# tmuird/VAEUNET

Measured on AMD Instinct MI355X. Metric: images/sec (whole node) at 3x512x512 bs=8/GPU; Dice parity vs CPU ref, higher is better.
Workload: dtype bf16; 1 GPU; UNet(3,2) train step (fwd+CombinedLoss+bwd+clip+AdamW), random-init weights; image=3x512x512, batch_per_gpu=8, global_batch=8, parallelism=dp1, execution=hipgraph-replay, wgrad_side_stream=False

## Files before the change

include/vaeunet.h:

```cpp
#ifndef VAEUNET_H
#define VAEUNET_H
#include <stdint.h>
#ifdef __cplusplus
extern "C" {
#endif

typedef struct VuGather {
  const void* src[3];
  int64_t stride[3];
  int32_t cend[3];
  int32_t nsrc;
  int32_t C;
  int32_t N, H, W;
  int32_t Hs, Ws;
  int32_t R, S;
  int32_t sy, sx, dy, dx, oy, ox;
} VuGather;

typedef struct VuGemmFwd {
  VuGather a;
  const void* b;
  int64_t ldb;
  int32_t ncol;
  int32_t out_mode;
// ... 121 lines not shown
int64_t vu_permute4_chunk(void);
int64_t vu_permute4_tile(void);
int vu_permute4_batch(const VuPermJob* jobs, int njobs, int64_t nchunks,
                      void* stream);
int vu_permute4_batch2(const VuPermJob* jobs, int njobs, int ntap,
                       int64_t tap_blocks, int64_t rest_blocks, void* stream);

int vu_bn_finalize(const float* psum, const float* pm2, int tiles,
                   int64_t tile_rows, int64_t rows, int C,
                   const float* gamma, const float* beta,
                   float* running_mean, float* running_var, float momentum,
                   float eps, float* scale, float* shift, float* save_mean,
                   float* save_invstd, int64_t* num_batches_tracked,
                   float* workspace, void* stream);
int vu_bn_eval_coeffs(const float* gamma, const float* beta,
                      const float* running_mean, const float* running_var,
                      float eps, int C, float* scale, float* shift,
                      float* save_mean, float* save_invstd, void* stream);
int vu_bn_fwd_fused_supported(int tiles, int C, int64_t ys, int64_t rs, int64_t os);
int vu_bn_fwd_fused(const float* psum, const float* pm2, int tiles, int64_t tile_rows, int64_t P, int C,
                    const float* gamma, const float* beta, float* running_mean, float* running_var,
                    int64_t* num_batches_tracked, float momentum, float eps, float* coef, const void* y,
                    int64_t ys, const void* res, int64_t rs, const float* rscale, const float* rshift,
                    void* out, int64_t os, int relu, int dtype, void* stream);
int vu_bn_apply(const void* x, int64_t x_stride, void* y, int64_t y_stride,
                int64_t P, int C, const float* scale, const float* shift,
                int relu, int dtype, void* stream);
int vu_bn_bwd_fused_supported(int64_t P, int C, int64_t dys, int64_t xs, int64_t dxs);
int vu_bn_bwd_fused(const void* dy, int64_t dys, const void* x, int64_t xs, int64_t P, int C,
                    const float* scale, const float* shift, const float* mean, const float* invstd,
                    const float* gamma, int relu, int train, float* dgamma, float* dbeta,
                    int accumulate, void* dx, int64_t dxs, float* workspace, int dtype, void* stream);
int vu_bn_bwd_reduce(const void* dy, int64_t dy_stride, const void* x,
                     int64_t x_stride, int64_t P, int C, const float* scale,
                     const float* shift, const float* mean,
                     const float* invstd, const float* gamma, int relu,
                     int train, float* dgamma, float* dbeta, int accumulate,
                     float* coef, float* workspace, int dtype, void* stream);
int64_t vu_bn_bwd_finish_workspace_bytes(int nblk, int C);
int vu_bn_bwd_finish(const float* part, int nblk, int64_t P, int C,
                     const float* gamma, const float* invstd, int train,
                     float* dgamma, float* dbeta, int accumulate, float* coef,
                     float* workspace, void* stream);
int vu_bn_bwd_apply(const void* dy, int64_t dy_stride, const void* x,
                    int64_t x_stride, int64_t P, int C, const float* scale,
                    const float* shift, const float* mean, const float* coef,
                    int relu, void* dx, int64_t dx_stride, int dtype,
                    void* stream);
int vu_bn_bwd_apply2_ok(int C, int64_t dys, int64_t x1s, int64_t x2s, int64_t dx1s, int64_t dx2s);
int vu_bn_bwd_apply2(const void* dy, int64_t dys, const void* x1, int64_t x1s, const void* x2, int64_t x2s,
                     int64_t P, int C, const float* mean1, const float* coef1, const float* mean2,
                     const float* coef2, void* dx1, int64_t dx1s, void* dx2, int64_t dx2s, int dtype,
                     void* stream);

int vu_chan_sum(const void* x, int64_t stride, int N, int H, int W, int y0,
                int x0, int Hr, int Wr, int C, float* out, int accumulate,
                float* workspace, int dtype, void* stream);
int64_t vu_reduce_workspace_bytes(int64_t P, int C);
int64_t vu_bn_finalize_workspace_bytes(int tiles, int C);
int vu_zero(void* y, int64_t ys, int64_t P, int C, int dtype, void* stream);
int vu_gpu_delay(int rounds, void* stream);
int vu_zero_insert2(const void* dy, int64_t dys, int N, int h, int w, int C,
                    void* up, int64_t ups, int H, int W, int dtype, void* stream);
int vu_copy(const void* x, int64_t xs, int xdtype, void* y, int64_t ys,
            int ydtype, int64_t P, int C, int accumulate, void* stream);
int vu_input_pack(const float* x, int64_t sn, int64_t sc, int64_t sh,
                  int64_t sw, int N, int C, int H, int W, int Cp, void* y,
                  int dtype, void* stream);

int vu_maxpool2_fwd(const void* x, int64_t xs, int N, int H, int W, int C,
                    void* y, int64_t ys, int dtype, void* stream);
int vu_maxpool2_bwd(const void* x, int64_t xs, const void* dy, int64_t dys,
                    int N, int H, int W, int C, void* dx, int64_t dxs,
                    const void* add, int64_t adds, int dtype, void* stream);
int vu_bn_apply_maxpool2(const void* y, int64_t ys, void* a, int64_t as, void* pool, int64_t ps,
                         int N, int H, int W, int C, const float* scale, const float* shift,
                         int relu, int dtype, void* stream);
int vu_bn_bwd_pool_supported(int H, int W, int C, int64_t ys, int64_t dps, int64_t adds, int64_t dxs);
int vu_bn_bwd_pool(const void* y, int64_t ys, const void* dp, int64_t dps, const void* add, int64_t adds,
                   int N, int H, int W, int C, const float* scale, const float* shift, const float* mean,
                   const float* invstd, const float* gamma, int relu, int train, float* dgamma,
                   float* dbeta, int accumulate, float* coef, float* workspace, void* dx, int64_t dxs,
                   int dtype, void* stream);
int vu_upsample_fwd(const void* x, int64_t xs, int N, int Hi, int Wi, int C,
                    void* y, int64_t ys, int Ho, int Wo, int Hp, int Wp,
                    int py, int px, int dtype, void* stream);
int vu_upsample_bwd(const void* dy, int64_t dys, int N, int Hi, int Wi, int C,
                    void* dx, int64_t dxs, int Ho, int Wo, int Hp, int Wp,
                    int py, int px, int accumulate, int dtype, void* stream);

int64_t vu_attn_tile_rows(void);
int vu_attn_psi_fwd(const void* ug, const void* ux, int64_t P, int F,
                    const float* sg, const float* tg, const float* sx,
                    const float* tx, const float* wpsi, const float* bpsi,
                    float* q, float* psum, float* pm2, int64_t tile_rows,
                    int dtype, void* stream);
int vu_attn_gate_fwd(const float* q, const float* st, const void* x,
                     int64_t xs, int64_t P, int C, float* pmap, void* out,
                     int64_t os, int dtype, void* stream);
int vu_attn_gate_bwd(const void* dout, int64_t dos, const void* x, int64_t xs,
                     const float* pmap, int64_t P, int C, void* dx,
                     int64_t dxs, float* dqpre, int dtype, void* stream);
int64_t vu_attn_psi_bwd_workspace_bytes(int64_t P, int F);
int vu_attn_psi_bwd(const void* ug, const void* ux, int64_t P, int F,
                    const float* sg, const float* tg, const float* sx,
                    const float* tx, const float* wpsi, const float* dq,
// ... 256 lines not shown
```

vaeunet_amd/_lib.py:

```python
import ctypes as C
import os

import torch

_HERE = os.path.dirname(os.path.abspath(__file__))
LIB_PATH = os.path.join(_HERE, "libvaeunet_hip.so")
if os.environ.get("VU_LIB_PATH"):
    LIB_PATH = os.environ["VU_LIB_PATH"]

F32, BF16 = 0, 1

_p = C.c_void_p
_i = C.c_int
_l = C.c_int64
_f = C.c_float


class VuGather(C.Structure):
    _fields_ = [("src", _p * 3), ("stride", _l * 3), ("cend", C.c_int32 * 3),
                ("nsrc", C.c_int32), ("C", C.c_int32),
                ("N", C.c_int32), ("H", C.c_int32), ("W", C.c_int32),
                ("Hs", C.c_int32), ("Ws", C.c_int32), ("R", C.c_int32), ("S", C.c_int32),
                ("sy", C.c_int32), ("sx", C.c_int32), ("dy", C.c_int32), ("dx", C.c_int32),
                ("oy", C.c_int32), ("ox", C.c_int32)]
# ... 54 lines not shown
class VuLatentHeads(C.Structure):
    _fields_ = [("z", _p), ("eps", _p), ("logvar", _p), ("dmu_in", _p), ("dlv_in", _p), ("dz_in", _p), ("pooled", _p),
                ("w_mu", _p), ("w_lv", _p), ("dw_mu", _p), ("db_mu", _p), ("dw_lv", _p), ("db_lv", _p),
                ("dpooled", _p), ("C", C.c_int32), ("grad_acc", C.c_int32)]


_SIGS = {
    "vu_gemm_fwd": (_i, [C.POINTER(VuGemmFwd), _i, _p]),
    "vu_gemm_fwd_row_tile": (_l, [C.POINTER(VuGemmFwd), _i]),
    "vu_gemm_fwd_workspace_bytes": (_l, [C.POINTER(VuGemmFwd), _i]),
    "vu_gemm_fwd_bnb_tile": (_l, [C.POINTER(VuGemmFwd), _i]),
    "vu_gemm_fwd_kernel": (_i, [C.POINTER(VuGemmFwd), _i]),
    "vu_abi_struct_sizes": (None, [_p]),
    "vu_bn_bwd_finish": (_i, [_p, _i, _l, _i, _p, _p, _i, _p, _p, _i, _p, _p, _p]),
    "vu_bn_bwd_finish_workspace_bytes": (_l, [_i, _i]),
    "vu_gemm_wgrad": (_i, [C.POINTER(VuGemmWgrad), _i, _p]),
    "vu_gemm_wgrad_tile": (_i, [C.POINTER(VuGemmWgrad), _i, C.POINTER(C.c_int), C.POINTER(C.c_int)]),
    "vu_gemm_set_tuning": (_i, [_i, _i]),
    "vu_gemm_experiment_modes": (_i, []),
    "vu_slab_reduce": (_i, [_p, _i, _i, _i, _i, _i, _l, _l, _l, _p, _i, _p]),
    "vu_amax": (_i, [_p, _l, _l, _i, _p, _i, _i, _p]),
    "vu_quant_fp8": (_i, [_p, _l, _l, _i, _p, _p, _l, _p, _i, _p]),
    "vu_quant_rows_fp8": (_i, [_p, _i, _l, _p, _l, _p, _p]),
    "vu_bn_apply_fp8": (_i, [_p, _l, _p, _l, _l, _i, _p, _p, _i, _p, _i, _i, _p, _i, _p]),
    "vu_conv3x3_fp8_row_tile": (_l, [C.POINTER(VuConvFp8)]),
    "vu_conv3x3_fp8": (_i, [C.POINTER(VuConvFp8), _p]),
    "vu_conv3x3_fp8_workspace_bytes": (_l, [C.POINTER(VuConvFp8)]),
    "vu_conv3x3_fp8_minmax_ok": (_i, [C.POINTER(VuConvFp8)]),
    "vu_fp8_relu_amax": (_i, [_p, _p, _l, _i, _p, _p, _i, _p, _p]),
    "vu_permute4_chunk": (_l, []),
    "vu_permute4_tile": (_l, []),
    "vu_permute4_batch": (_i, [_p, _i, _l, _p]),
    "vu_permute4_batch2": (_i, [_p, _i, _i, _l, _l, _p]),
    "vu_permute4": (_i, [_p, _l, _l, _l, _l, _l, _i, _i, _i, _i, _i, _p, _i, _p]),
    "vu_bn_finalize": (_i, [_p, _p, _i, _l, _l, _i, _p, _p, _p, _p, _f, _f, _p, _p, _p, _p,
                            _p, _p, _p]),
    "vu_bn_finalize_workspace_bytes": (_l, [_i, _i]),
    "vu_bn_eval_coeffs": (_i, [_p, _p, _p, _p, _f, _i, _p, _p, _p, _p, _p]),
    "vu_bn_apply": (_i, [_p, _l, _p, _l, _l, _i, _p, _p, _i, _i, _p]),
    "vu_bn_fwd_fused_supported": (_i, [_i, _i, _l, _l, _l]),
    "vu_bn_bwd_fused_supported": (_i, [_l, _i, _l, _l, _l]),
    "vu_bn_bwd_fused": (_i, [_p, _l, _p, _l, _l, _i, _p, _p, _p, _p, _p, _i, _i, _p, _p, _i, _p, _l, _p, _i,
                             _p]),
    "vu_bn_fwd_fused": (_i, [_p, _p, _i, _l, _l, _i, _p, _p, _p, _p, _p, _f, _f, _p, _p, _l, _p, _l, _p, _p,
                             _p, _l, _i, _i, _p]),
    "vu_bn_bwd_pool_supported": (_i, [_i, _i, _i, _l, _l, _l, _l]),
    "vu_bn_bwd_pool": (_i, [_p, _l, _p, _l, _p, _l, _i, _i, _i, _i, _p, _p, _p, _p, _p, _i, _i, _p, _p, _i, _p, _p,
                            _p, _l, _i, _p]),
    "vu_bn_bwd_reduce": (_i, [_p, _l, _p, _l, _l, _i, _p, _p, _p, _p, _p, _i, _i, _p, _p, _i,
                              _p, _p, _i, _p]),
    "vu_bn_bwd_apply": (_i, [_p, _l, _p, _l, _l, _i, _p, _p, _p, _p, _i, _p, _l, _i, _p]),
    "vu_bn_bwd_apply2_ok": (_i, [_i, _l, _l, _l, _l, _l]),
    "vu_bn_bwd_apply2": (_i, [_p, _l, _p, _l, _p, _l, _l, _i, _p, _p, _p, _p, _p, _l, _p, _l, _i, _p]),
    "vu_reduce_workspace_bytes": (_l, [_l, _i]),
    "vu_chan_sum": (_i, [_p, _l, _i, _i, _i, _i, _i, _i, _i, _i, _p, _i, _p, _i, _p]),
    "vu_copy": (_i, [_p, _l, _i, _p, _l, _i, _l, _i, _i, _p]),
    "vu_zero": (_i, [_p, _l, _l, _i, _i, _p]),
    "vu_gpu_delay": (_i, [_i, _p]),
    "vu_zero_insert2": (_i, [_p, _l, _i, _i, _i, _i, _p, _l, _i, _i, _i, _p]),
    "vu_input_pack": (_i, [_p, _l, _l, _l, _l, _i, _i, _i, _i, _i, _p, _i, _p]),
    "vu_maxpool2_fwd": (_i, [_p, _l, _i, _i, _i, _i, _p, _l, _i, _p]),
    "vu_maxpool2_bwd": (_i, [_p, _l, _p, _l, _i, _i, _i, _i, _p, _l, _p, _l, _i, _p]),
    "vu_bn_apply_maxpool2": (_i, [_p, _l, _p, _l, _p, _l, _i, _i, _i, _i, _p, _p, _i, _i, _p]),
    "vu_upsample_fwd": (_i, [_p, _l, _i, _i, _i, _i, _p, _l, _i, _i, _i, _i, _i, _i, _i, _p]),
    "vu_upsample_bwd": (_i, [_p, _l, _i, _i, _i, _i, _p, _l, _i, _i, _i, _i, _i, _i, _i, _i,
                             _p]),
    "vu_attn_tile_rows": (_l, []),
    "vu_attn_psi_fwd": (_i, [_p, _p, _l, _i, _p, _p, _p, _p, _p, _p, _p, _p, _p, _l, _i, _p]),
    "vu_attn_gate_fwd": (_i, [_p, _p, _p, _l, _l, _i, _p, _p, _l, _i, _p]),
    "vu_attn_gate_bwd": (_i, [_p, _l, _p, _l, _p, _l, _i, _p, _l, _p, _i, _p]),
    "vu_attn_psi_bwd_workspace_bytes": (_l, [_l, _i]),
    "vu_attn_psi_bwd_blocks": (_l, [_l]),
    "vu_attn_psi_bwd_bnb_ok": (_i, [_i]),
    "vu_attn_psi_bwd_bnb": (_i, [_p, _p, _l, _i, _p, _p, _p, _p, _p, _p, _p, _p, _p, _i, _p, _p, _p, _p, _p, _p, _p,
                                 _i, _p]),
    "vu_attn_psi_bwd": (_i, [_p, _p, _l, _i, _p, _p, _p, _p, _p, _p, _p, _p, _p, _i, _p, _i,
                             _p]),
    "vu_attn_tail_bwd_tile": (_l, [_i, _i]),
    "vu_attn_tail_bwd_ok": (_i, [_l, _i, _i, _l, _l, _l, _l, _l, _l, _i]),
    "vu_attn_tail_bwd": (_i, [_p, _p, _p, _l, _i, _i, _p, _p, _p, _p, _p, _p, _p, _p, _p, _p, _l, _p, _l, _p, _l,
                              _p, _p, _l, _l, _i, _p, _l, _p, _p, _i, _p]),
    "vu_pointwise_fwd": (_i, [_p, _l, _l, _i, _i, _p, _p, _p, _l, _i, _p]),
    "vu_pointwise_bwd_workspace_bytes": (_l, [_l, _i, _i]),
    "vu_pointwise_bn_fwd": (_i, [_p, _l, _l, _i, _i, _p, _p, _p, _p, _p, _l, _i, _p]),
    "vu_pointwise_bn_bwd_blocks": (_l, [_l]),
    "vu_pointwise_bn_bwd": (_i, [_p, _l, _p, _l, _p, _l, _l, _i, _i, _p, _p, _l, _p, _p, _i, _p, _p, _i, _p]),
    "vu_pointwise_bwd": (_i, [_p, _l, _p, _l, _l, _i, _i, _p, _p, _l, _p, _p, _i, _p, _i, _p]),
    "vu_loss_workspace_bytes": (_l, []),
    "vu_bce_dice_fwd2": (_i, [_p, _p, _l, _p, _f, _f, _f, _p, _p, _p, _p]),
    "vu_bce_dice_bwd": (_i, [_p, _p, _l, _p, _f, _f, _f, _p, _p, _p]),
    "vu_kl_free_bits2": (_i, [_p, _p, _i, _i, _f, _p, _p, _p, _p, _p]),
    "vu_sumsq": (_i, [_p, _l, _p, _p, _p]),
    "vu_dice_score": (_i, [_p, _p, _l, _f, _p, _p, _p, _p]),
    "vu_seg_counts_workspace_bytes": (_l, [_l]),
    "vu_seg_counts": (_i, [_p, _i, C.POINTER(_l), _i, _i, _p, _i, C.POINTER(_l), _i, _i, _i, _i, _i, _i, _p, _i, _p,
                           _p, _p]),
    "vu_seg_metrics": (_i, [_p, _i, _i, C.c_double, _p, _p, _i, _p, _p]),
    "vu_calib_workspace_bytes": (_l, []),
    "vu_calib_hist": (_i, [_p, _p, _i, _p, _l, _i, _f, _p, _p, _p, _p, _p, _p, _i, _p, _p]),
    "vu_calib_metrics": (_i, [_p, _p, _i, _p, _p, _p, _p, _p, _p, _p]),
    "vu_mt_chunk_elems": (_l, []),
    "vu_mt_grad_norm": (_i, [_p, _i, _l, _f, _p, _p, _p, _p]),
    "vu_mt_scale_grads": (_i, [_p, _i, _l, _p, _p]),
    "vu_mt_adamw": (_i, [_p, _i, _l, _f, _f, _f, _f, _f, _p, _p]),
    "vu_mt_adamw_dev": (_i, [_p, _i, _l, C.c_double, C.c_double, C.c_double, C.c_double, C.c_double, _p, _i,
                             _p]),
# ... 78 lines not shown
```

vaeunet_amd/csrc/bn.hip:

```cpp
#include <cstdlib>
#include <type_traits>

#include "host.h"

namespace {

constexpr int STATS_TPB = 32;
constexpr int STATS_MAXS = 256;

__global__ void bn_stats_stage1(const float* psum, const float* pm2, int tiles, int64_t tile_rows,
                                int64_t rows, int C, int S, double* ws) {
  __shared__ double sh[4][64];
  const int cl = threadIdx.x & 63, tl = threadIdx.x >> 6;
  const int c = blockIdx.x * 64 + cl;
  const bool ok = c < C;
  const int per = (tiles + S - 1) / S;
  const int tb0 = blockIdx.y * per, te0 = min(tiles, tb0 + per);
  constexpr int U = STATS_TPB / 4;
  double N = 0, Mn = 0, Q = 0;
  for (int tb = tb0; tb < te0; tb += STATS_TPB) {
    const int te = min(te0, tb + STATS_TPB);
    const int64_t n_r = min(rows, (int64_t)te * tile_rows) - (int64_t)tb * tile_rows;
    float sv[U], mv[U];
    double nv[U];
    const int cc = ok ? c : 0;
#pragma unroll
    for (int u = 0; u < U; ++u) {
      const int t = min(tb + tl + 4 * u, te - 1);
      sv[u] = psum[(int64_t)t * C + cc];
      mv[u] = pm2[(int64_t)t * C + cc];
    }
#pragma unroll
    for (int u = 0; u < U; ++u) {
      const int t = tb + tl + 4 * u;
      const bool in = ok && t < te;
      sv[u] = in ? sv[u] : 0.f;
      mv[u] = in ? mv[u] : 0.f;
      int64_t nt = rows - (int64_t)t * tile_rows;
      nv[u] = in ? (double)(nt > tile_rows ? tile_rows : nt) : 0.0;
    }
    double s = 0;
#pragma unroll
    for (int u = 0; u < U; ++u) s += (double)sv[u];
    sh[tl][cl] = s;
    __syncthreads();
    const double m = (sh[0][cl] + sh[1][cl] + sh[2][cl] + sh[3][cl]) / (double)n_r;
    __syncthreads();
    double q = 0;
#pragma unroll
    for (int u = 0; u < U; ++u) {
      if (nv[u] > 0) {
        const double d = (double)sv[u] / nv[u] - m;
        q += (double)mv[u] + nv[u] * d * d;
      }
    }
    sh[tl][cl] = q;
// ... 268 lines not shown
                             const float* invstd, float* dgamma, float* dbeta, int accumulate,
                             float* coef, int train) {
  int c = blockIdx.x * 32 + (threadIdx.x & 31);
  const int cl = c < C ? c : C - 1;
  const float g = gamma ? gamma[cl] : 1.f;
  const float is = invstd[cl];
  const float dg0 = (dgamma && accumulate) ? dgamma[cl] : 0.f;
  const float db0 = (dbeta && accumulate) ? dbeta[cl] : 0.f;
  double s[2];
  colsum32<2>(part, nblk, 2 * (int64_t)C, C, c, c < C, s);
  if (threadIdx.x >= 32 || c >= C) return;
  float k1 = g * is;
  coef[c] = k1;
  coef[C + c] = train ? (float)(-(double)k1 * is * s[1] / (double)P) : 0.f;
  coef[2 * C + c] = train ? (float)(-(double)k1 * s[0] / (double)P) : 0.f;
  if (dgamma) dgamma[c] = accumulate ? dg0 + (float)s[1] : (float)s[1];
  if (dbeta) dbeta[c] = accumulate ? db0 + (float)s[0] : (float)s[0];
}

template <typename T, bool NT>
__global__ __launch_bounds__(256) void bn_bwd_apply_kernel(const T* dy, int64_t dys, const T* x, int64_t xs, int64_t P, int C,
                                    const float* scale, const float* shift, const float* mean,
                                    const float* coef, int relu, T* dx, int64_t dxs) {
  ChanMap cm(C);
  const int c = cm.cv * 8;
  float sc[8], sf[8], mu[8], k1[8], k2[8], k3[8];
#pragma unroll
  for (int i = 0; i < 8; ++i) {
    sc[i] = scale[c + i]; sf[i] = shift[c + i]; mu[i] = mean[c + i];
    k1[i] = coef[c + i]; k2[i] = coef[C + c + i]; k3[i] = coef[2 * C + c + i];
  }
  const int64_t step = (int64_t)gridDim.x * cm.R * UNR;
  for (int64_t p0 = (int64_t)blockIdx.x * cm.R * UNR + cm.row; p0 < P; p0 += step) {
    Vec8<T> vd[UNR], vx[UNR];
#pragma unroll
    for (int u = 0; u < UNR; ++u) {
      const int64_t p = p0 + (int64_t)u * cm.R;
      if (p < P) {
        if (NT) {
          vd[u].load_nt(dy + p * dys + c);
          vx[u].load_nt(x + p * xs + c);
        } else {
          vd[u].load(dy + p * dys + c);
          vx[u].load(x + p * xs + c);
        }
      }
    }
#pragma unroll
    for (int u = 0; u < UNR; ++u) {
      const int64_t p = p0 + (int64_t)u * cm.R;
      if (p >= P) continue;
      Vec8<T> vo;
#pragma unroll
      for (int i = 0; i < 8; ++i) {
        float xv = vx[u].get(i), dz = vd[u].get(i);
        if (relu && !(fmaf(xv, sc[i], sf[i]) > 0.f)) dz = 0.f;
        vo.set(i, fmaf(k1[i], dz, k2[i] * (xv - mu[i])) + k3[i]);
      }
      vo.store(dx + p * dxs + c);
    }
  }
}

template <typename T, bool NT>
__global__ __launch_bounds__(256) void bn_bwd_apply2_kernel(const T* dy, int64_t dys, const T* x1, int64_t x1s, const T* x2, int64_t x2s,
                                     int64_t P, int C, const float* mean1, const float* coef1, const float* mean2,
                                     const float* coef2, T* dx1, int64_t dx1s, T* dx2, int64_t dx2s) {
  ChanMap cm(C);
  const int c = cm.cv * 8;
  float mu1[8], a1[8], b1[8], e1[8], mu2[8], a2[8], b2[8], e2[8];
#pragma unroll
  for (int i = 0; i < 8; ++i) {
    mu1[i] = mean1[c + i]; a1[i] = coef1[c + i]; b1[i] = coef1[C + c + i]; e1[i] = coef1[2 * C + c + i];
    mu2[i] = mean2[c + i]; a2[i] = coef2[c + i]; b2[i] = coef2[C + c + i]; e2[i] = coef2[2 * C + c + i];
  }
  const int64_t step = (int64_t)gridDim.x * cm.R * UNR;
  for (int64_t p0 = (int64_t)blockIdx.x * cm.R * UNR + cm.row; p0 < P; p0 += step) {
    Vec8<T> vd[UNR], v1[UNR], v2[UNR];
#pragma unroll
    for (int u = 0; u < UNR; ++u) {
      const int64_t p = p0 + (int64_t)u * cm.R;
      if (p < P) {
        if (NT) {
          vd[u].load_nt(dy + p * dys + c);
          v1[u].load_nt(x1 + p * x1s + c);
          v2[u].load_nt(x2 + p * x2s + c);
        } else {
          vd[u].load(dy + p * dys + c);
          v1[u].load(x1 + p * x1s + c);
          v2[u].load(x2 + p * x2s + c);
        }
      }
    }
#pragma unroll
    for (int u = 0; u < UNR; ++u) {
      const int64_t p = p0 + (int64_t)u * cm.R;
      if (p >= P) continue;
      Vec8<T> o1, o2;
#pragma unroll
      for (int i = 0; i < 8; ++i) {
        const float dz = vd[u].get(i);
        o1.set(i, fmaf(a1[i], dz, b1[i] * (v1[u].get(i) - mu1[i])) + e1[i]);
        o2.set(i, fmaf(a2[i], dz, b2[i] * (v2[u].get(i) - mu2[i])) + e2[i]);
      }
      o1.store(dx1 + p * dx1s + c);
      o2.store(dx2 + p * dx2s + c);
    }
  }
}

template <typename T>
// ... 916 lines not shown
```

vaeunet_amd/engine.py:

```python
import warnings

import torch

from . import kernels as K
from ._lib import BF16, F32


OVERLAP_WGRAD = False

FUSE_BN_BWD_REDUCE = True


class SideStream:

    _per_device = {}

    def __init__(self, device):
        self.stream = torch.cuda.Stream(device=device)
        self.keep = []
        self.pending = False

    @classmethod
    def get(cls, device):
        key = torch.device(device).index
# ... 354 lines not shown
    return dx


def bn_bwd_pair(dy, a, b, M):
    outs, ks = [], []
    for x, coef, bn, part in (a, b):
        gw, gb, acc = bn_grad_sinks(bn)
        ks.append(K.bn_backward_finish(part, x, coef, bn.weight, gw, gb, acc, train=bn.training))
        outs.append(torch.empty_like(x))
    (xa, ca, _, _), (xb, cb, _, _) = a, b
    if not K.bn_backward_apply2(dy, xa, ca, ks[0], outs[0], xb, cb, ks[1], outs[1], K.dcode(xa.dtype)):
        K._apply(dy, xa, ca, ks[0], False, outs[0], K.dcode(xa.dtype), None)
        K._apply(dy, xb, cb, ks[1], False, outs[1], K.dcode(xb.dtype), None)
    return outs[0], outs[1]


FOLD_BN_EVAL = True


def can_fold(M, bn):
    return FOLD_BN_EVAL and M.infer and not bn.training and bn.track_running_stats \
        and bn.running_mean is not None


def fold_bn_eval(M, conv, bn, cin_pad=None, cin_use=None):
    co = conv.out_channels
    coef = bn_coef(bn, None, co)
    img = w3x3_fwd(conv.weight, F32, cin_pad, cin_use)
    w = img * coef[0][:, None]
    if M.d != F32:
        w = w.to(torch.bfloat16)
    b = coef[1] if conv.bias is None else conv.bias.float() * coef[0] + coef[1]
    return w, b.contiguous()


def conv_bn_relu_fwd(M, srcs, conv, bn, cin_pad=None, defer=False, zbias=None, cin_use=None):
    N, _, H, W = srcs[0].shape
    co = conv.out_channels
    if can_fold(M, bn) and not defer:
        wf, bf = fold_bn_eval(M, conv, bn, cin_pad, cin_use)
        a = M.act(N, co, H, W)
        K.gemm_fwd(K.gather3x3(srcs), wf, co, a, M.d, bias=bf, relu=True, zbias=zbias)
        return a, None
    y = M.act(N, co, H, W)
    st = K.gemm_fwd(K.gather3x3(srcs), w3x3_fwd(conv.weight, M.d, cin_pad, cin_use), co, y, M.d,
                    stats=bn.training, zbias=zbias)
    if defer == "any" or (defer and K.pool_fusable(y)):
        return None, (y, bn_coef(bn, st, co))
    a = M.act(N, co, H, W)
    coef = bn_fwd_apply(bn, st, y, a, True, M)
    return a, (y, coef)


def conv_bn_relu_bwd(M, srcs, conv, bn, saved, da, need_dsrc, cvalid=None, dsrc=None, dsrc_acc=False,
                     cin_pad=None, da_part=None, feeds=None, shortcut=None):
    y, coef = saved
    zrs = shortcut.regions(y) if shortcut is not None else None
    dy = bn_bwd(da, y, coef, bn, True, M, part=da_part, zrs=zrs)
    if shortcut is not None:
        shortcut.dy = dy

    def wg():
        wgrad3x3(dy, srcs, conv.weight, M, cvalid, sink=shortcut.sink if shortcut is not None else None)
        M.notify([bn.weight, bn.bias] + ([conv.weight] if shortcut is None else []))
    M.side(wg, dy, *srcs)
    if not need_dsrc:
        return None
    N, _, H, W = y.shape
    cin = shortcut.lead if shortcut is not None else (cin_pad or conv.in_channels)
    if dsrc is None:
        dsrc = M.act(N, cin, H, W)
    bnb = None
    if feeds is not None and FUSE_BN_BWD_REDUCE:
        (fy, fcoef), fbn = feeds
        bnb = (fy, fcoef, True)
    wd = w3x3_dgrad(conv.weight, M.d, rows_use=cin) if shortcut is not None else w3x3_dgrad(conv.weight, M.d, cin)
    part = K.gemm_fwd(K.gather3x3([dy]), wd, cin, dsrc, M.d, accumulate=dsrc_acc, kind="dgrad", bnb=bnb)
    if feeds is not None:
        return dsrc, part
    return dsrc


def double_conv_fwd(M, seq, srcs, cin_pad=None, defer=False):
    conv1, bn1, _, conv2, bn2, _ = seq
    a1, s1 = conv_bn_relu_fwd(M, srcs, conv1, bn1, cin_pad)
    a2, s2 = conv_bn_relu_fwd(M, [a1], conv2, bn2, defer=defer)
    return a2, (srcs, a1, s1, s2)


def double_conv_bwd(M, seq, saved, da2, need_dsrc, cvalid=None, da2_part=None):
    conv1, bn1, _, conv2, bn2, _ = seq
    srcs, a1, s1, s2 = saved
    da1, part = conv_bn_relu_bwd(M, [a1], conv2, bn2, s2, da2, True, feeds=(s1, bn1), da_part=da2_part)
    return conv_bn_relu_bwd(M, srcs, conv1, bn1, s1, da1, need_dsrc, cvalid, da_part=part)


def down_fwd(M, mod, x, pend=None, defer=False):
    seq = mod.maxpool_conv[1].double_conv
    if x is None:
        y, coef = pend
        N, C_, H, W = y.shape
        x = M.act(N, C_, H, W)
        xp = M.act(N, C_, H // 2, W // 2)
        K.bn_apply_maxpool(y, x, xp, coef, True, M.d)
    else:
        xp = K.maxpool_fwd(x, M.d)
    out, sdc = double_conv_fwd(M, seq, [xp], defer=defer)
    return x, out, (x, sdc)


def down_bwd(M, mod, saved, dout, add=None):
    x, sdc = saved
    seq = mod.maxpool_conv[1].double_conv
    dxp = double_conv_bwd(M, seq, sdc, dout, True)
    return PoolGrad(dxp, add, x)

# ... 260 lines not shown
```

vaeunet_amd/kernels.py:

```python
import ctypes as C

import torch

from . import _lib
from ._lib import ptr, call, query, stream, VuGather, VuGemmFwd, VuGemmWgrad

CL = torch.channels_last


def dcode(dtype):
    if dtype == torch.bfloat16:
        return _lib.BF16
    if dtype == torch.float32:
        return _lib.F32
    raise TypeError(f"unsupported activation dtype {dtype}")


def empty_act(N, Cc, H, W, dtype, device):
    return torch.empty((N, Cc, H, W), dtype=dtype, device=device, memory_format=CL)


def zeros_act(N, Cc, H, W, dtype, device):
    y = torch.empty((N, Cc, H, W), dtype=dtype, device=device, memory_format=CL)
    zero(y)
# ... 458 lines not shown
    N, Cc, H, W = x.shape
    P = N * H * W
    dev = x.device
    ws = torch.empty(query("vu_reduce_workspace_bytes", P, Cc) // 4 + 1, dtype=torch.float32,
                     device=dev)
    if fused and query("vu_bn_bwd_fused_supported", P, Cc, pstride(dy), pstride(x), pstride(dx)):
        call("vu_bn_bwd_fused", ptr(dy), pstride(dy), ptr(x), pstride(x), P, Cc, ptr(coef[0]), ptr(coef[1]),
             ptr(coef[2]), ptr(coef[3]), ptr(gamma), 1 if relu else 0, 1 if train else 0, ptr(dgamma), ptr(dbeta),
             1 if acc else 0, ptr(dx), pstride(dx), ptr(ws), dtype, stream())
        return dx
    k = torch.empty((3, Cc), dtype=torch.float32, device=dev)
    call("vu_bn_bwd_reduce", ptr(dy), pstride(dy), ptr(x), pstride(x), P, Cc, ptr(coef[0]),
         ptr(coef[1]), ptr(coef[2]), ptr(coef[3]), ptr(gamma), 1 if relu else 0,
         1 if train else 0, ptr(dgamma), ptr(dbeta), 1 if acc else 0, ptr(k), ptr(ws), dtype,
         stream())
    _apply(dy, x, coef, k, relu, dx, dtype, zrs)
    return dx


def bn_backward_pool(dp, add, y, coef, gamma, relu, dgamma, dbeta, acc, dx, dtype, train=True):
    N, Cc, H, W = y.shape
    P = N * H * W
    ws = workspace_f32(query("vu_reduce_workspace_bytes", P, Cc), y.device)
    k = torch.empty((3, Cc), dtype=torch.float32, device=y.device)
    call("vu_bn_bwd_pool", ptr(y), pstride(y), ptr(dp), pstride(dp), ptr(add), pstride(add) if add is not None else 0,
         N, H, W, Cc, ptr(coef[0]), ptr(coef[1]), ptr(coef[2]), ptr(coef[3]), ptr(gamma), 1 if relu else 0,
         1 if train else 0, ptr(dgamma), ptr(dbeta), 1 if acc else 0, ptr(k), ptr(ws), ptr(dx), pstride(dx),
         dtype, stream())
    return dx


def bn_backward_part(part, dy, x, coef, gamma, relu, dgamma, dbeta, acc, dx, dtype, train=True, zrs=None):
    N, Cc, H, W = x.shape
    P = N * H * W
    k = torch.empty((3, Cc), dtype=torch.float32, device=x.device)
    nb = query("vu_bn_bwd_finish_workspace_bytes", part.nblk, Cc)
    ws = workspace_f32(nb, x.device) if nb > 0 else None
    call("vu_bn_bwd_finish", ptr(part.part), part.nblk, P, Cc, ptr(gamma), ptr(coef[3]), 1 if train else 0,
         ptr(dgamma), ptr(dbeta), 1 if acc else 0, ptr(k), ptr(ws), stream())
    _apply(dy, x, coef, k, relu, dx, dtype, zrs)
    return dx


def bn_backward_finish(part, x, coef, gamma, dgamma, dbeta, acc, train=True):
    N, Cc, H, W = x.shape
    k = torch.empty((3, Cc), dtype=torch.float32, device=x.device)
    nb = query("vu_bn_bwd_finish_workspace_bytes", part.nblk, Cc)
    ws = workspace_f32(nb, x.device) if nb > 0 else None
    call("vu_bn_bwd_finish", ptr(part.part), part.nblk, N * H * W, Cc, ptr(gamma), ptr(coef[3]), 1 if train else 0,
         ptr(dgamma), ptr(dbeta), 1 if acc else 0, ptr(k), ptr(ws), stream())
    return k


def bn_backward_apply2(dy, x1, coef1, k1, dx1, x2, coef2, k2, dx2, dtype):
    N, Cc, H, W = x1.shape
    if not query("vu_bn_bwd_apply2_ok", Cc, pstride(dy), pstride(x1), pstride(x2), pstride(dx1), pstride(dx2)):
        return False
    call("vu_bn_bwd_apply2", ptr(dy), pstride(dy), ptr(x1), pstride(x1), ptr(x2), pstride(x2), N * H * W, Cc,
         ptr(coef1[2]), ptr(k1), ptr(coef2[2]), ptr(k2), ptr(dx1), pstride(dx1), ptr(dx2), pstride(dx2), dtype,
         stream())
    return True


def chan_sum(x, out, acc, dtype, window=None):
    N, Cc, H, W = x.shape
    y0, x0, Hr, Wr = window if window is not None else (0, 0, H, W)
    ws = torch.empty(query("vu_reduce_workspace_bytes", N * Hr * Wr, Cc) // 4 + 1,
                     dtype=torch.float32, device=x.device)
    call("vu_chan_sum", ptr(x), pstride(x), N, H, W, y0, x0, Hr, Wr, Cc, ptr(out),
         1 if acc else 0, ptr(ws), dtype, stream())


def zero(y):
    N, Cc, H, W = y.shape
    call("vu_zero", ptr(y), pstride(y), N * H * W, Cc, dcode(y.dtype), stream())


def copy(x, y, accumulate=False):
    N, Cc, H, W = x.shape
    call("vu_copy", ptr(x), pstride(x), dcode(x.dtype), ptr(y), pstride(y), dcode(y.dtype),
         N * H * W, Cc, 1 if accumulate else 0, stream())


def input_pack(x, Cp, dtype):
    N, Cc, H, W = x.shape
    if x.dtype != torch.float32:
        x = x.float()
    y = empty_act(N, Cp, H, W, torch.bfloat16 if dtype == _lib.BF16 else torch.float32, x.device)
    s = x.stride()
    call("vu_input_pack", ptr(x), s[0], s[1], s[2], s[3], N, Cc, H, W, Cp, ptr(y), dtype, stream())
    return y


def maxpool_fwd(x, dtype):
    N, Cc, H, W = x.shape
    y = empty_act(N, Cc, H // 2, W // 2, x.dtype, x.device)
    call("vu_maxpool2_fwd", ptr(x), pstride(x), N, H, W, Cc, ptr(y), pstride(y), dtype, stream())
    return y


def maxpool_bwd(x, dy, dx, add, dtype):
    N, Cc, H, W = x.shape
    call("vu_maxpool2_bwd", ptr(x), pstride(x), ptr(dy), pstride(dy), N, H, W, Cc, ptr(dx),
         pstride(dx), ptr(add), pstride(add) if add is not None else 0, dtype, stream())
    return dx

# ... 34 lines not shown
```

Baseline: 575.8 images/sec.

## Fuse BN backward apply into first-layer image conv weight-gradient kernel

Adds a dedicated MFMA weight-gradient kernel for the first 3x3 conv (8-channel padded image input, 64 outputs). It recomputes the BN backward elementwise result on the fly from da and y, so the full-resolution dy tensor is never written and re-read. The BN reduction still runs separately beforehand, and partial results go into per-block slabs that are then reduced. A shared bn_bwd_elem helper turns off FP contraction to keep results consistent with the existing apply kernel. The fused path adds a new kernel whose efficiency is not known, along with a slab reduction step.

```diff
diff --git a/include/vaeunet.h b/include/vaeunet.h
--- a/include/vaeunet.h
+++ b/include/vaeunet.h
@@ -197,6 +197,13 @@
                      int64_t P, int C, const float* mean1, const float* coef1, const float* mean2,
                      const float* coef2, void* dx1, int64_t dx1s, void* dx2, int64_t dx2s, int dtype,
                      void* stream);
+int vu_conv_image_wgrad_bn_ok(int C, int Cp, int64_t das, int64_t ys, int64_t imgs, int N, int H, int W,
+                              int dtype);
+int vu_conv_image_wgrad_bn_slabs(int N, int H, int W);
+int vu_conv_image_wgrad_bn(const void* da, int64_t das, const void* y, int64_t ys, const float* scale,
+                           const float* shift, const float* mean, const float* k, int relu,
+                           const void* img, int64_t imgs, int N, int H, int W, float* slab, int nslab,
+                           void* stream);
 
 int vu_chan_sum(const void* x, int64_t stride, int N, int H, int W, int y0,
                 int x0, int Hr, int Wr, int C, float* out, int accumulate,
diff --git a/vaeunet_amd/_lib.py b/vaeunet_amd/_lib.py
--- a/vaeunet_amd/_lib.py
+++ b/vaeunet_amd/_lib.py
@@ -130,6 +130,9 @@
     "vu_bn_bwd_apply": (_i, [_p, _l, _p, _l, _l, _i, _p, _p, _p, _p, _i, _p, _l, _i, _p]),
     "vu_bn_bwd_apply2_ok": (_i, [_i, _l, _l, _l, _l, _l]),
     "vu_bn_bwd_apply2": (_i, [_p, _l, _p, _l, _p, _l, _l, _i, _p, _p, _p, _p, _p, _l, _p, _l, _i, _p]),
+    "vu_conv_image_wgrad_bn_ok": (_i, [_i, _i, _l, _l, _l, _i, _i, _i, _i]),
+    "vu_conv_image_wgrad_bn_slabs": (_i, [_i, _i, _i]),
+    "vu_conv_image_wgrad_bn": (_i, [_p, _l, _p, _l, _p, _p, _p, _p, _i, _p, _l, _i, _i, _i, _p, _i, _p]),
     "vu_reduce_workspace_bytes": (_l, [_l, _i]),
     "vu_chan_sum": (_i, [_p, _l, _i, _i, _i, _i, _i, _i, _i, _i, _p, _i, _p, _i, _p]),
     "vu_copy": (_i, [_p, _l, _i, _p, _l, _i, _l, _i, _i, _p]),
diff --git a/vaeunet_amd/csrc/bn.hip b/vaeunet_amd/csrc/bn.hip
--- a/vaeunet_amd/csrc/bn.hip
+++ b/vaeunet_amd/csrc/bn.hip
@@ -2,6 +2,7 @@
 #include <type_traits>
 
 #include "host.h"
+#include "bn_bwd_elem.h"
 
 namespace {
 
@@ -376,11 +377,8 @@
       if (p >= P) continue;
       Vec8<T> vo;
 #pragma unroll
-      for (int i = 0; i < 8; ++i) {
-        float xv = vx[u].get(i), dz = vd[u].get(i);
-        if (relu && !(fmaf(xv, sc[i], sf[i]) > 0.f)) dz = 0.f;
-        vo.set(i, fmaf(k1[i], dz, k2[i] * (xv - mu[i])) + k3[i]);
-      }
+      for (int i = 0; i < 8; ++i)
+        vo.set(i, bn_bwd_elem(vx[u].get(i), vd[u].get(i), relu, sc[i], sf[i], mu[i], k1[i], k2[i], k3[i]));
       vo.store(dx + p * dxs + c);
     }
   }
diff --git a/vaeunet_amd/csrc/bn_bwd_elem.h b/vaeunet_amd/csrc/bn_bwd_elem.h
--- /dev/null
+++ b/vaeunet_amd/csrc/bn_bwd_elem.h
@@ -0,0 +1,9 @@
+#pragma once
+#include "common.h"
+
+VU_DEV float bn_bwd_elem(float xv, float dz, int relu, float sc, float sf, float mu, float k1, float k2,
+                         float k3) {
+#pragma clang fp contract(off)
+  if (relu && !(fmaf(xv, sc, sf) > 0.f)) dz = 0.f;
+  return fmaf(k1, dz, k2 * (xv - mu)) + k3;
+}
diff --git a/vaeunet_amd/csrc/conv_image_wgrad.hip b/vaeunet_amd/csrc/conv_image_wgrad.hip
--- /dev/null
+++ b/vaeunet_amd/csrc/conv_image_wgrad.hip
@@ -0,0 +1,232 @@
+#include "host.h"
+#include "bn_bwd_elem.h"
+
+namespace {
+
+typedef __attribute__((address_space(3))) s16x4 lds_s16x4;
+
+constexpr int NT = 256, NW = NT / 64;
+constexpr int TP = 32;
+constexpr int CO = 64;
+constexpr int NJ = 72, NJP = 80;
+constexpr int DYS = CO * 2 + 16;
+constexpr int PTS = NJP * 2;
+constexpr int WAVE_LDS = TP * (DYS + PTS);
+constexpr int NA = CO / 16, NB = NJP / 16;
+constexpr int RED = NA * NB * 4 * 64;
+constexpr int SMEM = (NW - 1) * RED * 4 > NW * WAVE_LDS ? (NW - 1) * RED * 4 : NW * WAVE_LDS;
+
+struct WgArgs {
+  const bf16_t* da;
+  int64_t das;
+  const bf16_t* y;
+  int64_t ys;
+  const float *scale, *shift, *mean, *k;
+  int relu;
+  const bf16_t* img;
+  int64_t imgs;
+  int N, H, W;
+  float* slab;
+};
+
+struct Tile {
+  u32x4 d[4], y[4];
+};
+
+VU_DEV u32x4 tr_frag(const char* lo, const char* hi) {
+  const s16x4 l = __builtin_amdgcn_ds_read_tr16_b64_v4i16((lds_s16x4*)lo);
+  const s16x4 h = __builtin_amdgcn_ds_read_tr16_b64_v4i16((lds_s16x4*)hi);
+  const u32x2 l2 = __builtin_bit_cast(u32x2, l), h2 = __builtin_bit_cast(u32x2, h);
+  return u32x4{l2[0], l2[1], h2[0], h2[1]};
+}
+
+template <bool BN>
+__global__ __launch_bounds__(NT, 2) void conv_image_wgrad_kernel(WgArgs a) {
+  __shared__ __attribute__((aligned(16))) char smem[SMEM];
+  const int lane = threadIdx.x & 63;
+  const int wid = __builtin_amdgcn_readfirstlane(threadIdx.x >> 6);
+  char* dyb = smem + wid * WAVE_LDS;
+  char* ptb = dyb + TP * DYS;
+  const int H = a.H, W = a.W, HW = a.H * a.W;
+  const int P = a.N * HW;
+  const int ntiles = (P + TP - 1) / TP;
+  const int c8 = lane & 7, r8 = lane >> 3;
+  const int c = c8 * 8;
+  const int tp = lane & 31, th = lane >> 5;
+  const FastDiv div_hw((uint32_t)HW), div_w((uint32_t)W);
+
+  float sc[8], sf[8], mu[8], k1[8], k2[8], k3[8];
+  if constexpr (BN) {
+#pragma unroll
+    for (int e = 0; e < 8; ++e) {
+      sc[e] = a.scale[c + e]; sf[e] = a.shift[c + e]; mu[e] = a.mean[c + e];
+      k1[e] = a.k[c + e]; k2[e] = a.k[CO + c + e]; k3[e] = a.k[2 * CO + c + e];
+    }
+  }
+
+  auto load_tile = [&](int t, Tile& q) {
+    const int p0 = t * TP;
+#pragma unroll
+    for (int i = 0; i < 4; ++i) {
+      const int p = min(p0 + i * 8 + r8, P - 1);
+      q.d[i] = __builtin_nontemporal_load(reinterpret_cast<const u32x4*>(a.da + (int64_t)p * a.das + c));
+      if constexpr (BN)
+        q.y[i] = __builtin_nontemporal_load(reinterpret_cast<const u32x4*>(a.y + (int64_t)p * a.ys + c));
+    }
+  };
+  auto load_taps = [&](int t, u32x4* tv) {
+    const int p0 = t * TP;
+    const bool ok = p0 + tp < P;
+    const int p = ok ? p0 + tp : P - 1;
+    const int n = (int)div_hw.div((uint32_t)p);
+    const int rem = p - n * HW;
+    const int h = (int)div_w.div((uint32_t)rem), w = rem - h * W;
+#pragma unroll
+    for (int j = 0; j < 5; ++j) {
+      const int tap = th * 5 + j;
+      const int ty = tap / 3;
+      const int yy = h + ty - 1, xx = w + (tap - ty * 3) - 1;
+      tv[j] = u32x4{0, 0, 0, 0};
+      if (ok && tap < 9 && (unsigned)yy < (unsigned)H && (unsigned)xx < (unsigned)W)
+        tv[j] = *reinterpret_cast<const u32x4*>(a.img + ((int64_t)(n * H + yy) * W + xx) * a.imgs);
+    }
+  };
+
+  f32x4 acc[NA][NB];
+#pragma unroll
+  for (int i = 0; i < NA; ++i)
+#pragma unroll
+    for (int j = 0; j < NB; ++j) acc[i][j] = f32x4{0, 0, 0, 0};
+
+  const int g4 = lane >> 4, li = lane & 15, qd = li >> 2, pp = li & 3;
+  const char* rdA = dyb + (8 * g4 + qd) * DYS + 8 * pp;
+  const char* rdB = ptb + (8 * g4 + qd) * PTS + 8 * pp;
+
+  auto store_taps = [&](const u32x4* tv) {
+#pragma unroll
+    for (int j = 0; j < 5; ++j) *reinterpret_cast<u32x4*>(ptb + tp * PTS + (th * 5 + j) * 16) = tv[j];
+  };
+
+  auto process = [&](int t, const Tile& q, const u32x4* tn, bool more) {
+    const int p0 = t * TP;
+#pragma unroll
+    for (int i = 0; i < 4; ++i) {
+      Vec8<bf16_t> vo;
+      if constexpr (BN) {
+        Vec8<bf16_t> vx, vd;
+        vx.v = q.y[i];
+        vd.v = q.d[i];
+#pragma unroll
+        for (int e = 0; e < 8; ++e)
+          vo.set(e, bn_bwd_elem(vx.get(e), vd.get(e), a.relu, sc[e], sf[e], mu[e], k1[e], k2[e], k3[e]));
+      } else {
+        vo.v = q.d[i];
+      }
+      if (p0 + i * 8 + r8 >= P) vo.zero();
+      *reinterpret_cast<u32x4*>(dyb + (i * 8 + r8) * DYS + c8 * 16) = vo.v;
+    }
+    asm volatile("" ::: "memory");
+    u32x4 af[NA], bf[NB];
+#pragma unroll
+    for (int i = 0; i < NA; ++i) af[i] = tr_frag(rdA + i * 32, rdA + 4 * DYS + i * 32);
+#pragma unroll
+    for (int j = 0; j < NB; ++j) bf[j] = tr_frag(rdB + j * 32, rdB + 4 * PTS + j * 32);
+    asm volatile("" ::: "memory");
+    if (more) store_taps(tn);
+#pragma unroll
+    for (int i = 0; i < NA; ++i)
+#pragma unroll
+      for (int j = 0; j < NB; ++j)
+        acc[i][j] = __builtin_amdgcn_mfma_f32_16x16x32_bf16(__builtin_bit_cast(bf16x8, af[i]),
+                                                            __builtin_bit_cast(bf16x8, bf[j]), acc[i][j], 0, 0, 0);
+  };
+
+  const int tstep = gridDim.x * NW;
+  int t = blockIdx.x * NW + wid;
+  if (t < ntiles) {
+    Tile cur;
+    u32x4 tn[5];
+    load_tile(t, cur);
+    load_taps(t, tn);
+    store_taps(tn);
+    for (; t < ntiles; t += tstep) {
+      Tile nxt;
+      const bool more = t + tstep < ntiles;
+      if (more) {
+        load_tile(t + tstep, nxt);
+        load_taps(t + tstep, tn);
+      }
+      process(t, cur, tn, more);
+      if (more) cur = nxt;
+    }
+  }
+
+  __syncthreads();
+  float* red = reinterpret_cast<float*>(smem);
+  if (wid > 0) {
+#pragma unroll
+    for (int i = 0; i < NA; ++i)
+#pragma unroll
+      for (int j = 0; j < NB; ++j)
+#pragma unroll
+        for (int r = 0; r < 4; ++r) red[(wid - 1) * RED + ((i * NB + j) * 4 + r) * 64 + lane] = acc[i][j][r];
+  }
+  __syncthreads();
+  if (wid != 0) return;
+#pragma unroll 1
+  for (int w = 0; w < NW - 1; ++w)
+#pragma unroll
+    for (int i = 0; i < NA; ++i)
+#pragma unroll
+      for (int j = 0; j < NB; ++j)
+#pragma unroll
+        for (int r = 0; r < 4; ++r) acc[i][j][r] += red[w * RED + ((i * NB + j) * 4 + r) * 64 + lane];
+  float* out = a.slab + (int64_t)blockIdx.x * CO * NJ;
+#pragma unroll
+  for (int i = 0; i < NA; ++i)
+#pragma unroll
+    for (int j = 0; j < NB; ++j) {
+      const int col = 16 * j + li;
+      if (col < NJ)
+#pragma unroll
+        for (int r = 0; r < 4; ++r) out[(16 * i + 4 * g4 + r) * NJ + col] = acc[i][j][r];
+    }
+}
+
+}
+
+extern "C" int vu_conv_image_wgrad_bn_ok(int C, int Cp, int64_t das, int64_t ys, int64_t imgs, int N, int H, int W,
+                                         int dtype) {
+  if (dtype != VU_BF16 || C != CO || Cp != 8) return 0;
+  if (das % 8 != 0 || ys % 8 != 0 || imgs % 8 != 0 || das < CO || ys < CO || imgs < 8) return 0;
+  if (N < 1 || H < 1 || W < 1) return 0;
+  if ((int64_t)N * H * W >= (int64_t)1 << 31) return 0;
+  return 1;
+}
+
+extern "C" int vu_conv_image_wgrad_bn_slabs(int N, int H, int W) {
+  const int64_t tiles = ((int64_t)N * H * W + TP - 1) / TP;
+  int64_t nblk = (tiles + NW - 1) / NW;
+  const int64_t cap = 2 * (int64_t)cu_count();
+  if (nblk > cap) nblk = cap;
+  return nblk < 1 ? 1 : (int)nblk;
+}
+
+extern "C" int vu_conv_image_wgrad_bn(const void* da, int64_t das, const void* y, int64_t ys, const float* scale,
+                                      const float* shift, const float* mean, const float* k, int relu,
+                                      const void* img, int64_t imgs, int N, int H, int W, float* slab, int nslab,
+                                      void* stream) {
+  if (!vu_conv_image_wgrad_bn_ok(CO, 8, das, y ? ys : das, imgs, N, H, W, VU_BF16)) return (int)hipErrorInvalidValue;
+  if (!da || !img || !slab || nslab < 1) return (int)hipErrorInvalidValue;
+  if (y && (!scale || !shift || !mean || !k)) return (int)hipErrorInvalidValue;
+  if ((reinterpret_cast<uintptr_t>(da) | reinterpret_cast<uintptr_t>(y) | reinterpret_cast<uintptr_t>(img)) % 16 != 0)
+    return (int)hipErrorInvalidValue;
+  WgArgs a{(const bf16_t*)da, das, (const bf16_t*)y, ys, scale, shift, mean, k, relu, (const bf16_t*)img, imgs,
+           N, H, W, slab};
+  hipStream_t st = (hipStream_t)stream;
+  if (y)
+    hipLaunchKernelGGL(conv_image_wgrad_kernel<true>, dim3((unsigned)nslab), dim3(NT), 0, st, a);
+  else
+    hipLaunchKernelGGL(conv_image_wgrad_kernel<false>, dim3((unsigned)nslab), dim3(NT), 0, st, a);
+  return (int)hipGetLastError();
+}
diff --git a/vaeunet_amd/engine.py b/vaeunet_amd/engine.py
--- a/vaeunet_amd/engine.py
+++ b/vaeunet_amd/engine.py
@@ -430,16 +430,58 @@
     return a, (y, coef)
 
 
+FUSE_IMAGE_WGRAD_BN = True
+
+
+def _image_wgrad_kernel_serves(M, srcs, conv, shortcut, da, y):
+    if not FUSE_IMAGE_WGRAD_BN or shortcut is not None or M.d != BF16 or K.AUDIT is not None:
+        return False
+    if len(srcs) != 1 or not conv.weight.requires_grad:
+        return False
+    return K.image_wgrad_bn_ok(da, y, srcs[0], M.d)
+
+
+def _image_wgrad_bn_serves(M, srcs, conv, bn, y, da, need_dsrc, da_part, shortcut):
+    if need_dsrc or isinstance(da, PoolGrad) or (da_part is not None and da_part.x is not y):
+        return False
+    N, Cc, H, W = y.shape
+    if da_part is None and FUSED_BN_BWD and K.query("vu_bn_bwd_fused_supported", N * H * W, Cc, K.pstride(da),
+                                                    K.pstride(y), Cc):
+        return False
+    return _image_wgrad_kernel_serves(M, srcs, conv, shortcut, da, y)
+
+
+def _image_wgrad_bn(M, srcs, conv, bn, y, coef, da, cvalid, da_part):
+    gw, gb, acc = bn_grad_sinks(bn)
+    if da_part is not None:
+        k = K.bn_backward_finish(da_part, y, coef, bn.weight, gw, gb, acc, train=bn.training)
+    else:
+        k = K.bn_backward_reduce(da, y, coef, bn.weight, True, gw, gb, acc, M.d, train=bn.training)
+
+    def wg():
+        g, gacc = grad_sink(conv.weight)
+        K.image_wgrad_bn(da, y, coef, k, True, srcs[0], g, conv_layout(g), gacc, cvalid=cvalid)
+        M.notify([bn.weight, bn.bias, conv.weight])
+    M.side(wg, da, y, k, *srcs)
+
+
 def conv_bn_relu_bwd(M, srcs, conv, bn, saved, da, need_dsrc, cvalid=None, dsrc=None, dsrc_acc=False,
                      cin_pad=None, da_part=None, feeds=None, shortcut=None):
     y, coef = saved
+    if _image_wgrad_bn_serves(M, srcs, conv, bn, y, da, need_dsrc, da_part, shortcut):
+        _image_wgrad_bn(M, srcs, conv, bn, y, coef, da, cvalid, da_part)
+        return None
     zrs = shortcut.regions(y) if shortcut is not None else None
     dy = bn_bwd(da, y, coef, bn, True, M, part=da_part, zrs=zrs)
     if shortcut is not None:
         shortcut.dy = dy
 
     def wg():
-        wgrad3x3(dy, srcs, conv.weight, M, cvalid, sink=shortcut.sink if shortcut is not None else None)
+        if _image_wgrad_kernel_serves(M, srcs, conv, shortcut, dy, dy):
+            g, gacc = grad_sink(conv.weight)
+            K.image_wgrad_bn(dy, None, None, None, False, srcs[0], g, conv_layout(g), gacc, cvalid=cvalid)
+        else:
+            wgrad3x3(dy, srcs, conv.weight, M, cvalid, sink=shortcut.sink if shortcut is not None else None)
         M.notify([bn.weight, bn.bias] + ([conv.weight] if shortcut is None else []))
     M.side(wg, dy, *srcs)
     if not need_dsrc:
diff --git a/vaeunet_amd/kernels.py b/vaeunet_amd/kernels.py
--- a/vaeunet_amd/kernels.py
+++ b/vaeunet_amd/kernels.py
@@ -534,6 +534,44 @@
     return k
 
 
+def bn_backward_reduce(dy, x, coef, gamma, relu, dgamma, dbeta, acc, dtype, train=True):
+    N, Cc, H, W = x.shape
+    P = N * H * W
+    ws = torch.empty(query("vu_reduce_workspace_bytes", P, Cc) // 4 + 1, dtype=torch.float32, device=x.device)
+    k = torch.empty((3, Cc), dtype=torch.float32, device=x.device)
+    call("vu_bn_bwd_reduce", ptr(dy), pstride(dy), ptr(x), pstride(x), P, Cc, ptr(coef[0]),
+         ptr(coef[1]), ptr(coef[2]), ptr(coef[3]), ptr(gamma), 1 if relu else 0,
+         1 if train else 0, ptr(dgamma), ptr(dbeta), 1 if acc else 0, ptr(k), ptr(ws), dtype,
+         stream())
+    return k
+
+
+def image_wgrad_bn_ok(da, y, img, dtype):
+    N, Cc, H, W = y.shape
+    return bool(query("vu_conv_image_wgrad_bn_ok", Cc, img.shape[1], pstride(da), pstride(y), pstride(img),
+                      N, H, W, dtype))
+
+
+def image_wgrad_bn(da, y, coef, k, relu, img, grad, layout, accumulate, cvalid=None, nslab=None):
+    N, _, H, W = img.shape
+    if nslab is None:
+        nslab = query("vu_conv_image_wgrad_bn_slabs", N, H, W)
+    slab = torch.empty((nslab, 64, 72), dtype=torch.float32, device=grad.device)
+    none = y is None
+
+    def launch():
+        call("vu_conv_image_wgrad_bn", ptr(da), pstride(da), ptr(y), 0 if none else pstride(y),
+             None if none else ptr(coef[0]), None if none else ptr(coef[1]), None if none else ptr(coef[2]),
+             None if none else ptr(k), 1 if relu else 0, ptr(img), pstride(img), N, H, W, ptr(slab), nslab,
+             stream())
+    _timed("conv3x3_image_wgrad", 2 * N * H * W * 64 * 72, launch, "conv_image_wgrad_kernel",
+           lambda: f"{N}x{H}x{W} 64x72 slabs {nslab}" + ("" if none else " bn"))
+    s_i, s_tap, s_c = layout
+    call("vu_slab_reduce", ptr(slab), nslab, 64, 72, 8, 8 if cvalid is None else cvalid, s_i, s_tap, s_c,
+         ptr(grad), 1 if accumulate else 0, stream())
+    return slab
+
+
 def bn_backward_apply2(dy, x1, coef1, k1, dx1, x2, coef2, k2, dx2, dtype):
     N, Cc, H, W = x1.shape
     if not query("vu_bn_bwd_apply2_ok", Cc, pstride(dy), pstride(x1), pstride(x2), pstride(dx1), pstride(dx2)):
```

Measured after the change: 581.7 images/sec (median of 6 runs). 1.01x the previous value.
